# beecave-homelab/VibeVoice-ROCm

Measured on AMD Instinct MI355X. Metric: audio-sec/s, higher is better.
Workload: dtype bf16; 1 GPU; cfg2: VibeVoice-1.5B shapes, 1 speaker(s) x 203-frame voice prompt, 330-token prompt, 225 frames (30.0 s audio), CFG=2.0, 20 DPM-Solver++ steps, whole generate() incl. voice encode + prefill; global_batch=1, parallelism=replicas x1 (one dialogue per GPU), hipgraph=True

## Files before the change

vibevoice_rocm_amd/csrc/vv_fused.hip:

```cpp
#include <hip/hip_runtime.h>
#include <stdint.h>

#include "vv_hip.h"
#include "vv_common.h"
#include "vv_device.h"

namespace {

__device__ __forceinline__ float bf2f(bf16_t v) { return __uint_as_float((unsigned)v << 16); }
__device__ __forceinline__ float ldw(const float* p) { return *p; }
__device__ __forceinline__ float ldw(const bf16_t* p) { return bf2f(*p); }

template <typename WT>
__global__ __launch_bounds__(256) void head_init_kernel(const WT* P, const float* noise, int D, int latent, float* Xs, float* Ms, float* h0, int64_t ldh) {
  extern __shared__ float nz[];
  for (int i = threadIdx.x; i < latent; i += blockDim.x) nz[i] = noise[i];
  __syncthreads();
  const int n = blockIdx.x * blockDim.x + threadIdx.x;
  if (n >= D + latent) return;
  float s;
  if (n < D) {
    s = 0.f;
    const WT* pr = P + (int64_t)n * latent;
    for (int j = 0; j < latent; ++j) s = fmaf(ldw(pr + j), nz[j], s);
    h0[n] = s;
    h0[ldh + n] = s;
  } else {
    s = nz[n - D];
  }
  Xs[n] = s;
  Ms[n] = 0.f;
}

template <typename WT>
__global__ __launch_bounds__(256) void head_sde_proj_kernel(const WT* P, const float* noise, int64_t ld_noise, int n_steps, int D, int latent, float* NX) {
  extern __shared__ float nz[];
  const int u = blockIdx.y, N = D + latent;
  const float* nr = noise + (int64_t)(u / n_steps) * ld_noise + (int64_t)(u % n_steps) * latent;
  for (int i = threadIdx.x; i < latent; i += blockDim.x) nz[i] = nr[i];
  __syncthreads();
  const int n = blockIdx.x * blockDim.x + threadIdx.x;
  if (n >= N) return;
  float s;
  if (n < D) {
    s = 0.f;
    const WT* pr = P + (int64_t)n * latent;
    for (int j = 0; j < latent; ++j) s = fmaf(ldw(pr + j), nz[j], s);
  } else {
    s = nz[n - D];
  }
  NX[(int64_t)u * N + n] = s;
}

struct BoundaryArgs {
  const float* G;
  const float* h; int64_t ldh;
  const float* shift; const float* scale; int64_t ld_mod;
  float eps, cfg;
  vv_dpm_coef k;
  float* Xs; float* Ms;
  float* h_out; int64_t ldh_out;
  float* latent_out;
  int D, latent;
  int64_t state_stride, latent_stride;
  const float* nx; int64_t nx_stride;
};

template <int KU, bool SDE>
__global__ __launch_bounds__(256) void head_boundary_kernel(BoundaryArgs a) {
#include "vv_head_boundary.inc"
}

template <int KU, bool SDE>
__global__ __launch_bounds__(256) void head_boundary_cfg_kernel(BoundaryArgs a, const float* __restrict__ cfg_rows) {
  a.cfg = cfg_rows[blockIdx.y];
#include "vv_head_boundary.inc"
}

template <int KU> void launch_boundary(const BoundaryArgs& a, int B, hipStream_t s, const float* cfg_rows) {
  const int n = a.D + a.latent;
  int blocks = (n + 3) / 4;
  if (blocks > 512) blocks = 512;
  if (B > 1 && blocks > 256) blocks = 256;
  if (cfg_rows) {
    if (a.nx) hipLaunchKernelGGL((head_boundary_cfg_kernel<KU, true>), dim3(blocks, B), dim3(256), 0, s, a, cfg_rows);
    else hipLaunchKernelGGL((head_boundary_cfg_kernel<KU, false>), dim3(blocks, B), dim3(256), 0, s, a, cfg_rows);
    return;
  }
  if (a.nx) hipLaunchKernelGGL((head_boundary_kernel<KU, true>), dim3(blocks, B), dim3(256), 0, s, a);
  else hipLaunchKernelGGL((head_boundary_kernel<KU, false>), dim3(blocks, B), dim3(256), 0, s, a);
}

enum { TAIL_ARGMAX = 0, TAIL_SAMPLE = 1, TAIL_ROWS = 2 };

template <typename WT, bool SAMPLE>
__global__ __launch_bounds__(256) void llm_tail_kernel(const float* h, int64_t ldh, int R, int H, const float* norm_w, float eps, float* out, int64_t ldo,
                                                       const WT* w_valid, int nv, const int* ids, float* logits_out, int* token_out, const int* forced,
                                                       int* lens, int tok_start, int tok_diff, int* frame_ctr, const vv_sampler smp, const float* q) {
  constexpr int MODE = SAMPLE ? TAIL_SAMPLE : TAIL_ARGMAX;
  const vv_sampler* samplers = nullptr;
  const uint64_t* seeds = nullptr;
#include "vv_llm_tail.inc"
}

template <typename WT>
__global__ __launch_bounds__(256) void llm_tail_rows_kernel(const float* h, int64_t ldh, int R, int H, const float* norm_w, float eps, float* out, int64_t ldo,
                                                            const WT* w_valid, int nv, const int* ids, float* logits_out, int* token_out, const int* forced,
                                                            int* lens, int tok_start, int tok_diff, int* frame_ctr, const vv_sampler* __restrict__ samplers,
                                                            const uint64_t* __restrict__ seeds) {
  constexpr int MODE = TAIL_ROWS;
  const vv_sampler smp = {1.f, 0, 1.f};
  const float* q = nullptr;
#include "vv_llm_tail.inc"
}

template <typename WT, bool SAMPLE>
__global__ __launch_bounds__(256) void llm_tail_fast_kernel(const float* h, int64_t ldh, int R, int H, const float* norm_w, float eps, float* out, int64_t ldo,
                                                            const WT* w_valid, int nv, const int* ids, float* logits_out, int* token_out, const int* forced,
                                                            int* lens, int tok_start, int tok_diff, int* frame_ctr, const int* active,
                                                            const vv_sampler smp, const float* q) {
  constexpr int MODE = SAMPLE ? TAIL_SAMPLE : TAIL_ARGMAX;
  const vv_sampler* samplers = nullptr;
  const uint64_t* seeds = nullptr;
#include "vv_llm_tail_fast.inc"
}

template <typename WT>
__global__ __launch_bounds__(256) void llm_tail_fast_rows_kernel(const float* h, int64_t ldh, int R, int H, const float* norm_w, float eps, float* out,
                                                                 int64_t ldo, const WT* w_valid, int nv, const int* ids, float* logits_out, int* token_out,
                                                                 const int* forced, int* lens, int tok_start, int tok_diff, int* frame_ctr, const int* active,
                                                                 const vv_sampler* __restrict__ samplers, const uint64_t* __restrict__ seeds) {
  constexpr int MODE = TAIL_ROWS;
  const vv_sampler smp = {1.f, 0, 1.f};
  const float* q = nullptr;
#include "vv_llm_tail_fast.inc"
}

struct CtxItem { float* pad; float* state; int ctx, T, C; const float* dw_w; float* hs; int affine; float scale, bias; };
struct CtxArgs { CtxItem it[VV_MAX_STAGES + 1 + 16]; int n; };

__global__ __launch_bounds__(256) void conv_ctx_gather_kernel(const CtxArgs a) {
  const CtxItem it = a.it[blockIdx.y];
  const int n = it.ctx * it.C;
  if (it.affine) {
    for (int i = blockIdx.x * 256 + threadIdx.x; i < n; i += gridDim.x * 256) it.pad[i] = fmaf(it.state[i], it.scale, it.bias);
    return;
  }
  for (int i = (blockIdx.x * 256 + threadIdx.x) * 4; i < n; i += gridDim.x * 1024) {
    if (i + 3 < n && (n & 3) == 0) *reinterpret_cast<float4*>(it.pad + i) = *reinterpret_cast<const float4*>(it.state + i);
    else for (int j = i; j < n && j < i + 4; ++j) it.pad[j] = it.state[j];
  }
}
__global__ __launch_bounds__(256) void conv_ctx_scatter_kernel(const CtxArgs a) {
  const CtxItem it = a.it[blockIdx.y];
  const int n = it.ctx * it.C;
  const float* src = it.pad + (int64_t)it.T * it.C;
  for (int i = (blockIdx.x * 256 + threadIdx.x) * 4; i < n; i += gridDim.x * 1024) {
    if (i + 3 < n && (n & 3) == 0 && (((int64_t)it.T * it.C) & 3) == 0) *reinterpret_cast<float4*>(it.state + i) = *reinterpret_cast<const float4*>(src + i);
    else for (int j = i; j < n && j < i + 4; ++j) it.state[j] = src[j];
  }
  if (it.hs) {
    for (int c = blockIdx.x * 256 + threadIdx.x; c < it.C; c += gridDim.x * 256) {
      float s = 0.f;
#pragma unroll
      for (int k = 0; k < 6; ++k) s = fmaf(it.dw_w[(size_t)c * 7 + k], src[(size_t)k * it.C + c], s);
      it.hs[c] = s;
    }
  }
}


struct AdaTab { const bf16_t* w[17]; float* out[17]; int nblk[17]; int ldo[17]; int n; };

typedef __bf16 ad_bf16x8 __attribute__((ext_vector_type(8)));
typedef unsigned int ad_u32x4 __attribute__((ext_vector_type(4)));

template <int NST, int NM>
__global__ __launch_bounds__(256) void adaln_all_kernel(const bf16_t* __restrict__ c, int rows, int D, const AdaTab tab) {
  __shared__ float red[4 * NM * 4 * 64];
  const int tid = threadIdx.x, lane = tid & 63, wave = tid >> 6;
  int bx = blockIdx.x, l = 0;
  while (l + 1 < tab.n && bx >= tab.nblk[l]) { bx -= tab.nblk[l]; ++l; }
  const int n0 = bx * 16, m0 = blockIdx.y * (16 * NM);
  const int r16 = lane & 15, kq = lane >> 4;
  const int kb = wave * (32 * NST) + 8 * kq;
  const bf16_t* wr = tab.w[l] + (int64_t)(n0 + r16) * D + kb;
  ad_u32x4 wf[NST], xf[NM][NST];
#pragma unroll
  for (int s = 0; s < NST; ++s) wf[s] = *reinterpret_cast<const ad_u32x4*>(wr + 32 * s);
#pragma unroll
  for (int t = 0; t < NM; ++t) {
    const bf16_t* xr = c + (int64_t)min(m0 + 16 * t + r16, rows - 1) * D + kb;
#pragma unroll
    for (int s = 0; s < NST; ++s) xf[t][s] = *reinterpret_cast<const ad_u32x4*>(xr + 32 * s);
  }
  f32x4 acc[NM];
#pragma unroll
  for (int t = 0; t < NM; ++t) acc[t] = f32x4{0.f, 0.f, 0.f, 0.f};
#pragma unroll
  for (int s = 0; s < NST; ++s)
#pragma unroll
    for (int t = 0; t < NM; ++t)
      acc[t] = __builtin_amdgcn_mfma_f32_16x16x32_bf16(__builtin_bit_cast(ad_bf16x8, wf[s]), __builtin_bit_cast(ad_bf16x8, xf[t][s]), acc[t], 0, 0, 0);
#pragma unroll
  for (int t = 0; t < NM; ++t)
#pragma unroll
    for (int i = 0; i < 4; ++i) red[((wave * NM + t) * 4 + i) * 64 + lane] = acc[t][i];
  __syncthreads();
  const int ei = tid >> 6, el = tid & 63;
  float* out = tab.out[l];
  const int ldo = tab.ldo[l];
#pragma unroll
  for (int t = 0; t < NM; ++t) {
    const int m = m0 + 16 * t + (el & 15);
    if (m < rows) {
      float v = 0.f;
#pragma unroll
      for (int w4 = 0; w4 < 4; ++w4) v += red[((w4 * NM + t) * 4 + ei) * 64 + el];
      out[(int64_t)m * ldo + n0 + 4 * (el >> 4) + ei] = v;
    }
  }
}

template <int NST>
__global__ __launch_bounds__(256) void adaln_lds_kernel(const bf16_t* __restrict__ c, int rows, const AdaTab tab, int total) {
  constexpr int D = 4 * 32 * NST, P = D + 8, NM = 3, RG = 40;
  extern __shared__ __attribute__((aligned(16))) unsigned char ad_smem[];
  bf16_t* xs = reinterpret_cast<bf16_t*>(ad_smem);
  const int tid = threadIdx.x, lane = tid & 63, wave = tid >> 6;
  const int m0 = blockIdx.y * RG;
  const int nr = min(RG, rows - m0);
  float* red = reinterpret_cast<float*>(ad_smem + (size_t)RG * P * 2);
  const int r16 = lane & 15, kq = lane >> 4;
// ... 165 lines not shown
      if (ch < KU * 128) {
        const float4 v = tv[r][c], w = nv[r][c];
        *reinterpret_cast<float4*>(&ys[r][ch * 4]) = ch < nchunks ? make_float4(v.x * rs * w.x, v.y * rs * w.y, v.z * rs * w.z, v.w * rs * w.w) : make_float4(0.f, 0.f, 0.f, 0.f);
      }
    }
  }
  asm volatile("s_waitcnt lgkmcnt(0)\n\ts_barrier" ::: "memory");
  float ya[KU][8], yb[KU][8];
#pragma unroll
  for (int u = 0; u < KU; ++u) {
#pragma unroll
    for (int h2 = 0; h2 < 2; ++h2) {
      const float4 p = *reinterpret_cast<const float4*>(&ys[0][u * 512 + lane * 8 + 4 * h2]), q = *reinterpret_cast<const float4*>(&ys[1][u * 512 + lane * 8 + 4 * h2]);
      ya[u][4 * h2] = p.x; ya[u][4 * h2 + 1] = p.y; ya[u][4 * h2 + 2] = p.z; ya[u][4 * h2 + 3] = p.w;
      yb[u][4 * h2] = q.x; yb[u][4 * h2 + 1] = q.y; yb[u][4 * h2 + 2] = q.z; yb[u][4 * h2 + 3] = q.w;
    }
  }
  for (int i = 0; i < rows_per_wave; ++i) {
    const int row = gw + i * nwaves;
    float sa = 0.f, sb = 0.f;
#pragma unroll
    for (int u = 0; u < KU; ++u) {
      const unsigned ua[4] = {wa[u].x, wa[u].y, wa[u].z, wa[u].w}, ub[4] = {wsm[u].x, wsm[u].y, wsm[u].z, wsm[u].w};
#pragma unroll
      for (int j = 0; j < 4; ++j) {
        sa = fmaf(__uint_as_float(ua[j] << 16), ya[u][2 * j], sa); sa = fmaf(__uint_as_float(ua[j] & 0xffff0000u), ya[u][2 * j + 1], sa);
        sb = fmaf(__uint_as_float(ub[j] << 16), yb[u][2 * j], sb); sb = fmaf(__uint_as_float(ub[j] & 0xffff0000u), yb[u][2 * j + 1], sb);
      }
    }
    if (i + 1 < rows_per_wave) issue(row + nwaves);
    sa = vv_wave_sum(sa);
    sb = vv_wave_sum(sb);
    if (lane == 0 && row < H) {
      const float v = (sa + a.b2_a[row]) + (sb + a.b2_s[row]);
      for (int r = 0; r < a.rows_out; ++r) a.out[(int64_t)r * a.ldo + row] = v;
    }
  }
}


struct HeadPreArgs {
  const bf16_t* Wc; const float* cond; int64_t ld_cond; int K;
  const float* temb; int n_steps; bf16_t* c_out;
  const bf16_t* P; const float* noise; int D, latent; float* Xs; float* Ms; float* h0; int64_t ldh;
  int gemv_blocks;
};

template <int KU>
__global__ __launch_bounds__(256) void head_pre_kernel(const HeadPreArgs a) {
  const int tid = threadIdx.x, lane = tid & 63, wave = tid >> 6;
  if ((int)blockIdx.x >= a.gemv_blocks) {
    __shared__ float nz[256];
    for (int i = tid; i < a.latent; i += 256) nz[i] = a.noise[i];
    __syncthreads();
    const int n = ((int)blockIdx.x - a.gemv_blocks) * 256 + tid;
    if (n >= a.D + a.latent) return;
    float s;
    if (n < a.D) {
      s = 0.f;
      const bf16_t* pr = a.P + (int64_t)n * a.latent;
      for (int j = 0; j < a.latent; ++j) s = fmaf(bf2f(pr[j]), nz[j], s);
      a.h0[n] = s;
      a.h0[a.ldh + n] = s;
    } else {
      s = nz[n - a.D];
    }
    a.Xs[n] = s;
    a.Ms[n] = 0.f;
    return;
  }
  const int D = a.D, npairs = D >> 1;
  const int nwaves = a.gemv_blocks * 4;
  int g = blockIdx.x * 4 + wave;
  float x[2][KU][8];
#pragma unroll
  for (int r = 0; r < 2; ++r)
#pragma unroll
    for (int u = 0; u < KU; ++u) {
      const float4 p = *reinterpret_cast<const float4*>(a.cond + r * a.ld_cond + u * 512 + lane * 8), q = *reinterpret_cast<const float4*>(a.cond + r * a.ld_cond + u * 512 + lane * 8 + 4);
      x[r][u][0] = p.x; x[r][u][1] = p.y; x[r][u][2] = p.z; x[r][u][3] = p.w; x[r][u][4] = q.x; x[r][u][5] = q.y; x[r][u][6] = q.z; x[r][u][7] = q.w;
    }
  for (; g < npairs; g += nwaves) {
    const int n = 2 * g;
    uint4 w[2][KU];
#pragma unroll
    for (int o = 0; o < 2; ++o)
#pragma unroll
      for (int u = 0; u < KU; ++u) w[o][u] = *reinterpret_cast<const uint4*>(a.Wc + (int64_t)(n + o) * a.K + u * 512 + lane * 8);
    float te[2][2];
#pragma unroll
    for (int ps = 0; ps < 2; ++ps) {
      const int i = min(lane + 64 * ps, a.n_steps - 1);
      const float2 t2 = *reinterpret_cast<const float2*>(a.temb + (int64_t)i * D + n);
      te[ps][0] = t2.x; te[ps][1] = t2.y;
    }
    float acc[2][2];
#pragma unroll
    for (int o = 0; o < 2; ++o) {
      acc[o][0] = 0.f; acc[o][1] = 0.f;
#pragma unroll
      for (int u = 0; u < KU; ++u) {
        const unsigned uu[4] = {w[o][u].x, w[o][u].y, w[o][u].z, w[o][u].w};
#pragma unroll
        for (int j = 0; j < 4; ++j) {
          const float w0 = __uint_as_float(uu[j] << 16), w1 = __uint_as_float(uu[j] & 0xffff0000u);
          acc[o][0] = fmaf(w0, x[0][u][2 * j], acc[o][0]); acc[o][0] = fmaf(w1, x[0][u][2 * j + 1], acc[o][0]);
          acc[o][1] = fmaf(w0, x[1][u][2 * j], acc[o][1]); acc[o][1] = fmaf(w1, x[1][u][2 * j + 1], acc[o][1]);
        }
      }
    }
    float c0[2][2];
#pragma unroll
    for (int o = 0; o < 2; ++o)
#pragma unroll
      for (int r = 0; r < 2; ++r) c0[o][r] = vv_wave_sum(acc[o][r]);
#pragma unroll
    for (int ps = 0; ps < 2; ++ps) {
      const int i = lane + 64 * ps;
      if (i < a.n_steps) {
#pragma unroll
        for (int r = 0; r < 2; ++r) {
          const float v0 = c0[0][r] + te[ps][0], v1 = c0[1][r] + te[ps][1];
          *reinterpret_cast<unsigned*>(a.c_out + ((int64_t)(i * 2 + r)) * D + n) = bf16_bits2(vv_silu(v0), vv_silu(v1));
        }
      }
    }
  }
}

}

int vv_head_init_fused(const vv_head* h, const float* noise, float* Xs, float* Ms, float* h0, int64_t ldh, hipStream_t s) {
  const int n = h->D + h->latent;
  const int blocks = (n + 255) / 256;
  const size_t lds = (size_t)h->latent * sizeof(float);
  if (h->wdt == VV_F32) hipLaunchKernelGGL((head_init_kernel<float>), dim3(blocks), dim3(256), lds, s, (const float*)h->noisy_proj, noise, h->D, h->latent, Xs, Ms, h0, ldh);
  else hipLaunchKernelGGL((head_init_kernel<bf16_t>), dim3(blocks), dim3(256), lds, s, (const bf16_t*)h->noisy_proj, noise, h->D, h->latent, Xs, Ms, h0, ldh);
  VV_CHECK_LAUNCH("vv_head_init_fused");
  return 0;
}

int vv_head_sde_proj_fused(const vv_head* h, const float* sde_noise, int64_t ld_sde, int n_steps, int B, float* NX, hipStream_t s) {
  const int n = h->D + h->latent;
  const dim3 grid((n + 255) / 256, B * n_steps);
  const size_t lds = (size_t)h->latent * sizeof(float);
  if (h->wdt == VV_F32)
    hipLaunchKernelGGL((head_sde_proj_kernel<float>), grid, dim3(256), lds, s, (const float*)h->noisy_proj, sde_noise, ld_sde, n_steps, h->D, h->latent, NX);
  else
    hipLaunchKernelGGL((head_sde_proj_kernel<bf16_t>), grid, dim3(256), lds, s, (const bf16_t*)h->noisy_proj, sde_noise, ld_sde, n_steps, h->D, h->latent, NX);
  VV_CHECK_LAUNCH("vv_head_sde_proj_fused");
  return 0;
}

bool vv_head_boundary_supported(const vv_head* h) {
  return h->fused_g != nullptr && h->D % 8 == 0 && h->D <= 4096 && ((uintptr_t)h->fused_g % 16 == 0);
}

int vv_head_boundary_decide(const vv_head* h) {
  const int ku = (h->D + 511) / 512;
  return (h->D > 0 && ku <= 8) ? ku : 0;
}

int vv_head_boundary_fused(const vv_head* h, const float* hrows, int64_t ldh, const float* shift, const float* scale, int64_t ld_mod, float cfg,
                           const vv_dpm_coef* k, float* Xs, float* Ms, float* h_out, int64_t ldh_out, float* latent_out, hipStream_t s) {
  return vv_head_boundary_batch(h, hrows, ldh, shift, scale, ld_mod, cfg, k, Xs, Ms, 0, h_out, ldh_out, latent_out, 0, 1, s);
}

int vv_head_boundary_batch(const vv_head* h, const float* hrows, int64_t ldh, const float* shift, const float* scale, int64_t ld_mod, float cfg,
                           const vv_dpm_coef* k, float* Xs, float* Ms, int64_t state_stride, float* h_out, int64_t ldh_out, float* latent_out,
                           int64_t latent_stride, int B, hipStream_t s, const float* nx, int64_t nx_stride, const float* cfg_rows) {
  BoundaryArgs a;
  a.state_stride = state_stride; a.latent_stride = latent_stride;
  a.nx = k->cn != 0.f ? nx : nullptr; a.nx_stride = nx_stride;
  a.G = h->fused_g; a.h = hrows; a.ldh = ldh; a.shift = shift; a.scale = scale; a.ld_mod = ld_mod; a.eps = h->eps; a.cfg = cfg; a.k = *k;
  a.Xs = Xs; a.Ms = Ms; a.h_out = h_out; a.ldh_out = ldh_out; a.latent_out = latent_out; a.D = h->D; a.latent = h->latent;
  switch (vv_head_boundary_decide(h)) {
    case 1: launch_boundary<1>(a, B, s, cfg_rows); break;
    case 2: launch_boundary<2>(a, B, s, cfg_rows); break;
    case 3: launch_boundary<3>(a, B, s, cfg_rows); break;
    case 4: launch_boundary<4>(a, B, s, cfg_rows); break;
    case 5: launch_boundary<5>(a, B, s, cfg_rows); break;
    case 6: launch_boundary<6>(a, B, s, cfg_rows); break;
    case 7: launch_boundary<7>(a, B, s, cfg_rows); break;
    case 8: launch_boundary<8>(a, B, s, cfg_rows); break;
    default: return vv_set_error(VV_E_UNSUPPORTED, "vv_head_boundary_fused: D=%d", h->D);
  }
  VV_CHECK_LAUNCH("vv_head_boundary_fused");
  return 0;
}

static int check_sampler(const char* name, const vv_sampler* smp, const float* q, int nv) {
  if (!smp || !q) return vv_set_error(VV_E_ARG, "%s: null sampler / q", name);
  if (!(smp->temperature > 0.f) || !(smp->top_p > 0.f && smp->top_p <= 1.f)) return vv_set_error(VV_E_ARG, "%s: temperature=%g (> 0) top_p=%g (0 < top_p <= 1)", name, (double)smp->temperature, (double)smp->top_p);
  if (nv > 8) return vv_set_error(VV_E_ARG, "%s: nv=%d (<= 8)", name, nv);
  return 0;
}

#define VV_TAIL_FAST(WT, SAMPLE, grid, R_, act)                                                                                                          \
  hipLaunchKernelGGL((llm_tail_fast_kernel<WT, SAMPLE>), dim3(grid), dim3(256), 0, s, h, ldh, R_, m->hidden, m->final_norm, m->rms_eps, out, ldo, (const WT*)w_valid, nv, \
                     ids, logits_out, token_out, forced_token, lens, tok_start, tok_diffusion, frame_counter, act, sv, q)
#define VV_TAIL_GEN(WT, SAMPLE)                                                                                                                         \
  hipLaunchKernelGGL((llm_tail_kernel<WT, SAMPLE>), dim3(1), dim3(256), lds, s, h, ldh, R, m->hidden, m->final_norm, m->rms_eps, out, ldo, (const WT*)w_valid, nv, ids, \
                     logits_out, token_out, forced_token, lens, tok_start, tok_diffusion, frame_counter, sv, q)
#define VV_TAIL_FAST_ROWS(WT, grid, R_, act)                                                                                                             \
  hipLaunchKernelGGL((llm_tail_fast_rows_kernel<WT>), dim3(grid), dim3(256), 0, s, h, ldh, R_, m->hidden, m->final_norm, m->rms_eps, out, ldo, (const WT*)w_valid, nv, \
                     ids, logits_out, token_out, forced_token, lens, tok_start, tok_diffusion, frame_counter, act, rows, seeds)
#define VV_TAIL_GEN_ROWS(WT)                                                                                                                            \
  hipLaunchKernelGGL((llm_tail_rows_kernel<WT>), dim3(1), dim3(256), lds, s, h, ldh, R, m->hidden, m->final_norm, m->rms_eps, out, ldo, (const WT*)w_valid, nv, ids, \
                     logits_out, token_out, forced_token, lens, tok_start, tok_diffusion, frame_counter, rows, seeds)

static int llm_tail_launch(const char* name, const vv_llm* m, const float* h, int64_t ldh, int R, float* out, int64_t ldo, const void* w_valid, int nv, const int* ids,
                           float* logits_out, int* token_out, const int* forced_token, int* lens, int tok_start, int tok_diffusion, int* frame_counter,
                           const vv_sampler* smp, const float* q, hipStream_t s, const vv_sampler* rows = nullptr, const uint64_t* seeds = nullptr) {
  const vv_sampler sv = smp ? *smp : vv_sampler{1.f, 0, 1.f};
  const size_t lds = (size_t)m->hidden * sizeof(float);
  auto a16 = [](const void* p) { return ((uintptr_t)p % 16) == 0; };
  if (R <= 2 && nv <= 8 && m->hidden % 4 == 0 && m->hidden <= 4096 && a16(h) && ldh % 4 == 0 && a16(out) && ldo % 4 == 0 && a16(m->final_norm) &&
      ((uintptr_t)w_valid % (m->wdt == VV_F32 ? 16 : 8)) == 0 && (m->wdt == VV_F32 || m->hidden % 4 == 0)) {
    if (rows) { if (m->wdt == VV_F32) VV_TAIL_FAST_ROWS(float, 1, R, (const int*)nullptr); else VV_TAIL_FAST_ROWS(bf16_t, 1, R, (const int*)nullptr); }
    else if (m->wdt == VV_F32) { if (smp) VV_TAIL_FAST(float, true, 1, R, (const int*)nullptr); else VV_TAIL_FAST(float, false, 1, R, (const int*)nullptr); }
    else { if (smp) VV_TAIL_FAST(bf16_t, true, 1, R, (const int*)nullptr); else VV_TAIL_FAST(bf16_t, false, 1, R, (const int*)nullptr); }
    VV_CHECK_LAUNCH(name);
    return 0;
  }
  if (rows) { if (m->wdt == VV_F32) VV_TAIL_GEN_ROWS(float); else VV_TAIL_GEN_ROWS(bf16_t); }
  else if (m->wdt == VV_F32) { if (smp) VV_TAIL_GEN(float, true); else VV_TAIL_GEN(float, false); }
  else { if (smp) VV_TAIL_GEN(bf16_t, true); else VV_TAIL_GEN(bf16_t, false); }
  VV_CHECK_LAUNCH(name);
  return 0;
}

static int llm_tail_batch_launch(const char* name, const vv_llm* m, const float* h, int64_t ldh, int B, float* out, int64_t ldo, const void* w_valid, int nv,
                                 const int* ids, float* logits_out, int* token_out, const int* forced_token, int* lens, int tok_start, int tok_diffusion,
                                 int* frame_counter, const int* active, const vv_sampler* smp, const float* q, hipStream_t s,
                                 const vv_sampler* rows = nullptr, const uint64_t* seeds = nullptr) {
  const vv_sampler sv = smp ? *smp : vv_sampler{1.f, 0, 1.f};
  auto a16 = [](const void* p) { return ((uintptr_t)p % 16) == 0; };
  if (!(m->hidden % 4 == 0 && m->hidden <= 4096 && a16(h) && ldh % 4 == 0 && a16(out) && ldo % 4 == 0 && a16(m->final_norm) &&
        ((uintptr_t)w_valid % (m->wdt == VV_F32 ? 16 : 8)) == 0))
    return vv_set_error(VV_E_UNSUPPORTED, "%s: hidden=%d / alignment not covered", name, m->hidden);
  if (rows) { if (m->wdt == VV_F32) VV_TAIL_FAST_ROWS(float, B, 2, active); else VV_TAIL_FAST_ROWS(bf16_t, B, 2, active); }
  else if (m->wdt == VV_F32) { if (smp) VV_TAIL_FAST(float, true, B, 2, active); else VV_TAIL_FAST(float, false, B, 2, active); }
  else { if (smp) VV_TAIL_FAST(bf16_t, true, B, 2, active); else VV_TAIL_FAST(bf16_t, false, B, 2, active); }
  VV_CHECK_LAUNCH(name);
  return 0;
}
#undef VV_TAIL_FAST
#undef VV_TAIL_GEN
#undef VV_TAIL_FAST_ROWS
#undef VV_TAIL_GEN_ROWS

extern "C" int vv_llm_tail(const vv_llm* m, const float* h, int64_t ldh, int R, float* out, int64_t ldo, const void* w_valid, int nv, const int* ids,
                           float* logits_out, int* token_out, const int* forced_token, int* lens, int tok_start, int tok_diffusion,
                           int* frame_counter, vv_stream_t stream) {
  if (!m || !h || !out || !w_valid || !ids || !logits_out || !token_out) return vv_set_error(VV_E_ARG, "vv_llm_tail: null pointer");
  if (R <= 0 || nv <= 0 || nv > 16) return vv_set_error(VV_E_ARG, "vv_llm_tail: R=%d nv=%d (nv <= 16)", R, nv);
  return llm_tail_launch("vv_llm_tail", m, h, ldh, R, out, ldo, w_valid, nv, ids, logits_out, token_out, forced_token, lens, tok_start, tok_diffusion, frame_counter,
                         nullptr, nullptr, (hipStream_t)stream);
}

extern "C" int vv_llm_tail_sample(const vv_llm* m, const float* h, int64_t ldh, int R, float* out, int64_t ldo, const void* w_valid, int nv, const int* ids,
                                  float* logits_out, int* token_out, const int* forced_token, int* lens, int tok_start, int tok_diffusion,
                                  int* frame_counter, const vv_sampler* sampler, const float* q, vv_stream_t stream) {
  if (!m || !h || !out || !w_valid || !ids || !logits_out || !token_out) return vv_set_error(VV_E_ARG, "vv_llm_tail_sample: null pointer");
  if (R <= 0 || nv <= 0) return vv_set_error(VV_E_ARG, "vv_llm_tail_sample: R=%d nv=%d", R, nv);
  VV_TRY(check_sampler("vv_llm_tail_sample", sampler, q, nv));
  return llm_tail_launch("vv_llm_tail_sample", m, h, ldh, R, out, ldo, w_valid, nv, ids, logits_out, token_out, forced_token, lens, tok_start, tok_diffusion,
                         frame_counter, sampler, q, (hipStream_t)stream);
}

extern "C" int vv_llm_tail_batch(const vv_llm* m, const float* h, int64_t ldh, int B, float* out, int64_t ldo, const void* w_valid, int nv, const int* ids,
                                 float* logits_out, int* token_out, const int* forced_token, int* lens, int tok_start, int tok_diffusion,
                                 int* frame_counter, const int* active, vv_stream_t stream) {
  if (!m || !h || !out || !w_valid || !ids || !logits_out || !token_out) return vv_set_error(VV_E_ARG, "vv_llm_tail_batch: null pointer");
  if (B <= 0 || B > 8 || nv <= 0 || nv > 8) return vv_set_error(VV_E_ARG, "vv_llm_tail_batch: B=%d (1..8) nv=%d (<= 8)", B, nv);
  return llm_tail_batch_launch("vv_llm_tail_batch", m, h, ldh, B, out, ldo, w_valid, nv, ids, logits_out, token_out, forced_token, lens, tok_start, tok_diffusion,
                               frame_counter, active, nullptr, nullptr, (hipStream_t)stream);
}

extern "C" int vv_llm_tail_batch_sample(const vv_llm* m, const float* h, int64_t ldh, int B, float* out, int64_t ldo, const void* w_valid, int nv, const int* ids,
                                        float* logits_out, int* token_out, const int* forced_token, int* lens, int tok_start, int tok_diffusion,
                                        int* frame_counter, const int* active, const vv_sampler* sampler, const float* q, vv_stream_t stream) {
  if (!m || !h || !out || !w_valid || !ids || !logits_out || !token_out) return vv_set_error(VV_E_ARG, "vv_llm_tail_batch_sample: null pointer");
  if (B <= 0 || B > 8 || nv <= 0) return vv_set_error(VV_E_ARG, "vv_llm_tail_batch_sample: B=%d (1..8) nv=%d", B, nv);
  VV_TRY(check_sampler("vv_llm_tail_batch_sample", sampler, q, nv));
  return llm_tail_batch_launch("vv_llm_tail_batch_sample", m, h, ldh, B, out, ldo, w_valid, nv, ids, logits_out, token_out, forced_token, lens, tok_start,
                               tok_diffusion, frame_counter, active, sampler, q, (hipStream_t)stream);
}

extern "C" int vv_llm_tail_sample_rows(const vv_llm* m, const float* h, int64_t ldh, int R, float* out, int64_t ldo, const void* w_valid, int nv, const int* ids,
                                       float* logits_out, int* token_out, const int* forced_token, int* lens, int tok_start, int tok_diffusion,
                                       int* frame_counter, const vv_sampler* samplers, const uint64_t* seeds, vv_stream_t stream) {
  if (!m || !h || !out || !w_valid || !ids || !logits_out || !token_out) return vv_set_error(VV_E_ARG, "vv_llm_tail_sample_rows: null pointer");
  if (R <= 0 || nv <= 0 || nv > 8) return vv_set_error(VV_E_ARG, "vv_llm_tail_sample_rows: R=%d nv=%d (<= 8)", R, nv);
  if (!lens || !samplers || !seeds) return vv_set_error(VV_E_ARG, "vv_llm_tail_sample_rows: null lens / samplers / seeds");
  return llm_tail_launch("vv_llm_tail_sample_rows", m, h, ldh, R, out, ldo, w_valid, nv, ids, logits_out, token_out, forced_token, lens, tok_start, tok_diffusion,
                         frame_counter, nullptr, nullptr, (hipStream_t)stream, samplers, seeds);
}

extern "C" int vv_llm_tail_batch_sample_rows(const vv_llm* m, const float* h, int64_t ldh, int B, float* out, int64_t ldo, const void* w_valid, int nv,
                                             const int* ids, float* logits_out, int* token_out, const int* forced_token, int* lens, int tok_start,
                                             int tok_diffusion, int* frame_counter, const int* active, const vv_sampler* samplers, const uint64_t* seeds,
                                             vv_stream_t stream) {
  if (!m || !h || !out || !w_valid || !ids || !logits_out || !token_out) return vv_set_error(VV_E_ARG, "vv_llm_tail_batch_sample_rows: null pointer");
  if (B <= 0 || B > 8 || nv <= 0 || nv > 8) return vv_set_error(VV_E_ARG, "vv_llm_tail_batch_sample_rows: B=%d (1..8) nv=%d (<= 8)", B, nv);
  if (!lens || !samplers || !seeds) return vv_set_error(VV_E_ARG, "vv_llm_tail_batch_sample_rows: null lens / samplers / seeds");
// ... 115 lines not shown
```

vibevoice_rocm_amd/csrc/vv_kernels.hip:

```cpp
#include <hip/hip_runtime.h>
#include <hip/hip_bf16.h>
#include <stdint.h>
#include <stdio.h>
#include <string.h>
#include <math.h>

#include "vv_hip.h"
#include "vv_common.h"
#include "vv_device.h"

static thread_local char g_err[512] = "";

int vv_set_error(int code, const char* fmt, ...) {
  va_list ap;
  va_start(ap, fmt);
  vsnprintf(g_err, sizeof(g_err), fmt, ap);
  va_end(ap);
  return code;
}

extern "C" const char* vv_last_error(void) { return g_err; }
extern "C" int vv_abi_version(void) { return 6; }
int vv_mixer_init();
extern "C" int vv_init(void) {
  VV_TRY(vv_mixer_init());
  VV_TRY(vv_mfma_gemm_init());
  VV_TRY(vv_gemm_packed_init());
  VV_TRY(vv_block1d_init());
  VV_TRY(vv_convffn_init());
  VV_TRY(vv_gemv_rows_init());
  return vv_fused_init();
}
static float* g_rows_part = nullptr;
static int* g_rows_tk = nullptr;
static const size_t G_ROWS_PART_FLOATS = (size_t)4 << 20, G_ROWS_TICKETS = 4096;
static int rows_scratch(int on) {
  if (on && !g_rows_part) {
    if (hipMalloc(&g_rows_part, G_ROWS_PART_FLOATS * sizeof(float)) != hipSuccess || hipMalloc(&g_rows_tk, G_ROWS_TICKETS * sizeof(int)) != hipSuccess ||
        hipMemset(g_rows_tk, 0, G_ROWS_TICKETS * sizeof(int)) != hipSuccess)
      return vv_set_error(VV_E_HIP, "vv_tune: gemv_rows_scratch allocation failed");
  }
  if (!on && g_rows_part) { (void)hipFree(g_rows_part); (void)hipFree(g_rows_tk); g_rows_part = nullptr; g_rows_tk = nullptr; }
  return 0;
}
void vv_gemv_rows_set_dbg(int d);
void vv_gemv_rows_set_atomic(int on);
void vv_gemv_stream_set_blocks(int b);
void vv_gemv_stream_set_waves(int w);
void vv_gemv_stream_set_opt(int o);
void vv_gemv_stream_set_long(int cap, int ku);
void vv_gemv_stream_set_dual_rw(int r);
void vv_gemv_stream_set_small_rw(int r);
void vv_mfma_set_mt(int mt);
void vv_mfma_set_tiled_rows(int r);
void vv_mfma_set_tiled_bk128(int on);
void vv_mfma_set_tiled_small(int t);
void vv_mfma_set_tiled_dual_bk64(int on);
void vv_mfma_set_tiled_small_dual(int t);
void vv_mfma_set_tiled_small_k(int k);
void vv_mixer_set_rows(int on);
void vv_mfma_set_mt_prefill(int mt);
extern int g_attn_group;
void vv_attn_decode_set_gqa(int on);
void vv_attn_decode_set_gqa_keys(int k);
extern "C" int vv_tune(const char* key, int value) {
  if (key && !strcmp(key, "gemv_long_cap")) { vv_gemv_stream_set_long(value, 0); return 0; }
  if (key && !strcmp(key, "gemv_long_ku")) { vv_gemv_stream_set_long(0, value); return 0; }
  if (key && !strcmp(key, "gemv_blocks")) { vv_gemv_stream_set_blocks(value); vv_gemv_mx6_set_blocks(value); return 0; }
  if (key && !strcmp(key, "gemv_waves")) { vv_gemv_stream_set_waves(value); return 0; }
  if (key && !strcmp(key, "gemv_rows")) { vv_gemv_rows_set(value, 0, -1); return 0; }
  if (key && !strcmp(key, "gemv_rows_blocks")) { vv_gemv_rows_set(-1, value, -1); return 0; }
  if (key && !strcmp(key, "gemv_rows_pers")) { vv_gemv_rows_set(-1, 0, value); return 0; }
  if (key && !strcmp(key, "gemv_rows_scratch")) return rows_scratch(value);
  if (key && !strcmp(key, "gemv_rows_dbg")) { vv_gemv_rows_set_dbg(value); return 0; }
  if (key && !strcmp(key, "gemv_rows_atomic")) { vv_gemv_rows_set_atomic(value); return 0; }
  if (key && !strcmp(key, "gemv_opt")) { vv_gemv_stream_set_opt(value); return 0; }
  if (key && !strcmp(key, "gemv_dual_rw")) { vv_gemv_stream_set_dual_rw(value); return 0; }
  if (key && !strcmp(key, "gemv_small_rw")) { vv_gemv_stream_set_small_rw(value); return 0; }
  if (key && !strcmp(key, "gemv_hot")) { vv_gemv_hot_set(value); return 0; }
  if (key && !strcmp(key, "conv_hot")) { vv_conv_hot_set(value); return 0; }
  if (key && !strcmp(key, "mixer_rows")) { vv_mixer_set_rows(value); return 0; }
  if (key && !strcmp(key, "block1d_fused")) { vv_block1d_set_fused(value); return 0; }
  if (key && !strcmp(key, "block1d_blocks")) { vv_block1d_set_blocks(value); return 0; }
  if (key && !strcmp(key, "convffn")) { vv_convffn_set(value); return 0; }
  if (key && !strcmp(key, "convffn_t1")) { vv_convffn_set_t1(value); return 0; }
  if (key && !strcmp(key, "convffn_t1hs")) { vv_convffn_set_t1hs(value); return 0; }
  if (key && !strcmp(key, "convffn_rows512")) { vv_convffn_set_rows(512, value); return 0; }
  if (key && !strcmp(key, "convffn_rows256")) { vv_convffn_set_rows(256, value); return 0; }
  if (key && !strcmp(key, "convffn_rows128")) { vv_convffn_set_rows(128, value); return 0; }
  if (key && !strcmp(key, "convffn_c128")) { vv_convffn_set_c128(value); return 0; }
  if (key && !strcmp(key, "skinny")) { vv_skinny_set(value, 0, 0); return 0; }
  if (key && !strcmp(key, "skinny_min_m")) { vv_skinny_set(1, value, 0); return 0; }
  if (key && !strcmp(key, "skinny_max_m")) { vv_skinny_set(1, 0, value); return 0; }
  if (key && !strcmp(key, "mfma_tiled_bk128")) { vv_mfma_set_tiled_bk128(value); return 0; }
  if (key && !strcmp(key, "attn_group")) { g_attn_group = value; return 0; }
  if (key && !strcmp(key, "attn_gqa")) { vv_attn_decode_set_gqa(value); return 0; }
  if (key && !strcmp(key, "attn_gqa_keys")) { vv_attn_decode_set_gqa_keys(value); return 0; }
  if (key && !strcmp(key, "mfma_tiled_small_k")) { vv_mfma_set_tiled_small_k(value); return 0; }
  if (key && !strcmp(key, "mfma_tiled_dual_bk64")) { vv_mfma_set_tiled_dual_bk64(value); return 0; }
  if (key && !strcmp(key, "mfma_tiled_small_dual")) { vv_mfma_set_tiled_small_dual(value); return 0; }
  if (key && !strcmp(key, "mfma_tiled_small")) { vv_mfma_set_tiled_small(value); return 0; }
  if (key && !strcmp(key, "mfma_tiled_rows")) { vv_mfma_set_tiled_rows(value); return 0; }
  if (key && !strcmp(key, "gemm_packed_rows")) { vv_gemm_packed_set_rows(value); return 0; }
  if (key && !strcmp(key, "mfma_mt")) { vv_mfma_set_mt(value); return 0; }
  if (key && !strcmp(key, "mfma_mt_prefill")) { vv_mfma_set_mt_prefill(value); return 0; }
  return vv_set_error(VV_E_ARG, "vv_tune: unknown key");
}

__device__ __forceinline__ float bf2f(unsigned int u16) { return __uint_as_float(u16 << 16); }
__device__ __forceinline__ float wave_sum(float v) {
#pragma unroll
  for (int o = 32; o > 0; o >>= 1) v += __shfl_xor(v, o);
  return v;
}

template <typename WT> struct WL;
template <> struct WL<float> {
  static __device__ __forceinline__ void load8(const float* p, float (&o)[8]) {
    const float4 a = *reinterpret_cast<const float4*>(p);
    const float4 b = *reinterpret_cast<const float4*>(p + 4);
    o[0] = a.x; o[1] = a.y; o[2] = a.z; o[3] = a.w; o[4] = b.x; o[5] = b.y; o[6] = b.z; o[7] = b.w;
  }
  static __device__ __forceinline__ void load4(const float* p, float (&o)[4]) {
    const float4 a = *reinterpret_cast<const float4*>(p);
    o[0] = a.x; o[1] = a.y; o[2] = a.z; o[3] = a.w;
  }
  static __device__ __forceinline__ float load1(const float* p) { return *p; }
};
template <> struct WL<bf16_t> {
  static __device__ __forceinline__ void load8(const bf16_t* p, float (&o)[8]) {
    const uint4 v = *reinterpret_cast<const uint4*>(p);
    unpack8(u32x4{v.x, v.y, v.z, v.w}, o);
  }
  static __device__ __forceinline__ void load4(const bf16_t* p, float (&o)[4]) {
    const uint2 v = *reinterpret_cast<const uint2*>(p);
    o[0] = __uint_as_float(v.x << 16); o[1] = __uint_as_float(v.x & 0xffff0000u);
    o[2] = __uint_as_float(v.y << 16); o[3] = __uint_as_float(v.y & 0xffff0000u);
  }
  static __device__ __forceinline__ float load1(const bf16_t* p) { return bf2f(*p); }
};

__device__ __forceinline__ void lin_epilogue(const vv_lin_args& a, int m, int n, float v, float v2) {
  a.out[(int64_t)m * a.ldo + n] = vv_epi_value(a, v, v2, EpiAtUse{a, m, n});
}

#define GEMV_THREADS 256

template <int M>
__device__ __forceinline__ void row_stats(const vv_lin_args& a, float* red, float (&rstd)[M]) {
  const int tid = threadIdx.x, lane = tid & 63, wave = tid >> 6;
  float ss[M];
#pragma unroll
  for (int m = 0; m < M; ++m) {
    const float* xr = a.x + (int64_t)m * a.ldx;
    float s = 0.f;
    for (int k = tid; k < a.k; k += GEMV_THREADS) { const float v = xr[k]; s += v * v; }
    ss[m] = wave_sum(s);
  }
  if (lane == 0) {
#pragma unroll
    for (int m = 0; m < M; ++m) red[wave * M + m] = ss[m];
  }
  __syncthreads();
#pragma unroll
  for (int m = 0; m < M; ++m) {
    const float t = red[m] + red[M + m] + red[2 * M + m] + red[3 * M + m];
    rstd[m] = rsqrtf(t / (float)a.k + a.eps);
  }
  __syncthreads();
}

template <int M>
__device__ __forceinline__ void stage_chunk(const vv_lin_args& a, float* xs, int kc0, int kc, int kcp, const float (&rstd)[M]) {
  for (int idx = threadIdx.x; idx < M * kcp; idx += GEMV_THREADS) {
    const int m = idx / kcp, kk = idx - m * kcp;
    float v = 0.f;
    if (kk < kc) {
      const int k = kc0 + kk;
      v = a.x[(int64_t)m * a.ldx + k];
      if (a.pro == VV_PRO_RMSNORM) {
        v *= rstd[m];
        if (a.norm_w) v *= a.norm_w[k];
        if (a.mod_scale) v = v * (1.0f + a.mod_scale[(int64_t)m * a.ld_mod + k]) + a.mod_shift[(int64_t)m * a.ld_mod + k];
      } else if (a.pro == VV_PRO_SILU) {
        v = vv_silu(v);
      }
    }
    xs[idx] = v;
  }
}

template <typename WT, int M, bool DUAL, int KSPLIT, int RW>
__global__ __launch_bounds__(GEMV_THREADS) void gemv_kernel(const vv_lin_args a, const int KC) {
  extern __shared__ __attribute__((aligned(16))) float smem[];
  float* red = smem;
  float* xs = smem + 64 * 4;
  const int tid = threadIdx.x, lane = tid & 63, wave = tid >> 6;
  const int K = a.k, N = a.n;
  const WT* __restrict__ W = reinterpret_cast<const WT*>(a.w);
  const WT* __restrict__ W2 = reinterpret_cast<const WT*>(a.w2);

  float rstd[M];
#pragma unroll
  for (int m = 0; m < M; ++m) rstd[m] = 1.f;
  if (a.pro == VV_PRO_RMSNORM) row_stats<M>(a, red, rstd);

  const int row0 = (KSPLIT == 1 ? (blockIdx.x * 4 + wave) : blockIdx.x) * RW;
  float acc[RW][M], acc2[DUAL ? RW : 1][M];
#pragma unroll
  for (int r = 0; r < RW; ++r)
#pragma unroll
    for (int m = 0; m < M; ++m) { acc[r][m] = 0.f; if (DUAL) acc2[r][m] = 0.f; }

  for (int kc0 = 0; kc0 < K; kc0 += KC) {
    const int kc = min(KC, K - kc0);
    const int kcp = (kc + 7) & ~7;
    if (kc0 > 0) __syncthreads();
    stage_chunk<M>(a, xs, kc0, kc, kcp, rstd);
    __syncthreads();
    const int kstart = (KSPLIT == 1 ? lane : (wave * 64 + lane)) * 8;
    const int kstep = (KSPLIT == 1 ? 64 : 256) * 8;
#pragma unroll 2
    for (int k = kstart; k < kc; k += kstep) {
      float w[RW][8], w2[DUAL ? RW : 1][8];
#pragma unroll
      for (int r = 0; r < RW; ++r) {
        const int n = min(row0 + r, N - 1);
        WL<WT>::load8(W + (int64_t)n * K + kc0 + k, w[r]);
        if (DUAL) WL<WT>::load8(W2 + (int64_t)n * K + kc0 + k, w2[r]);
      }
#pragma unroll
      for (int m = 0; m < M; ++m) {
        const float4 x0 = *reinterpret_cast<const float4*>(xs + m * kcp + k);
        const float4 x1 = *reinterpret_cast<const float4*>(xs + m * kcp + k + 4);
        const float xv[8] = {x0.x, x0.y, x0.z, x0.w, x1.x, x1.y, x1.z, x1.w};
#pragma unroll
        for (int r = 0; r < RW; ++r) {
#pragma unroll
          for (int j = 0; j < 8; ++j) {
            acc[r][m] = fmaf(w[r][j], xv[j], acc[r][m]);
            if (DUAL) acc2[r][m] = fmaf(w2[r][j], xv[j], acc2[r][m]);
          }
        }
      }
    }
  }
#pragma unroll
  for (int r = 0; r < RW; ++r)
#pragma unroll
    for (int m = 0; m < M; ++m) { acc[r][m] = wave_sum(acc[r][m]); if (DUAL) acc2[r][m] = wave_sum(acc2[r][m]); }
// ... 1776 lines not shown
```

Measured before the change: 44.07 audio-sec/s.

## Add multi-row specialized head boundary kernel for D=1536 single-batch CFG

Adds a specialized diffusion-head boundary kernel for D=1536, latent=64, B=1 with shared CFG and no SDE noise. Each wave computes two output rows and issues all of its weight loads before the RMSNorm/CFG stage. The grid is sized to exactly (D+latent)/8 blocks. The intent is to cut per-block fixed work and hide weight-load latency behind the normalization. In exchange it adds a shape-specific code path with more register pressure, and relies on the row count dividing evenly (1600/8=200).

```diff
diff --git a/vibevoice_rocm_amd/csrc/vv_fused.hip b/vibevoice_rocm_amd/csrc/vv_fused.hip
--- a/vibevoice_rocm_amd/csrc/vv_fused.hip
+++ b/vibevoice_rocm_amd/csrc/vv_fused.hip
@@ -77,8 +77,124 @@
 #include "vv_head_boundary.inc"
 }
 
+template <int R>
+__global__ __launch_bounds__(256) void head_boundary_rows_kernel(BoundaryArgs a) {
+  constexpr int KU = 3, NCH = (KU * 128 + 255) / 256;
+  __shared__ __attribute__((aligned(16))) float ys[KU * 512];
+  __shared__ float red[4][2];
+  const int tid = threadIdx.x, lane = tid & 63, wave = tid >> 6;
+  const int D = a.D;
+  const int nchunks = D >> 2;
+  float4 hv[2][NCH], sv[2][NCH], cv[2][NCH];
+#pragma unroll
+  for (int c = 0; c < NCH; ++c) {
+    const int ch = tid + c * 256;
+    const int kk = ch < nchunks ? ch * 4 : 0;
+#pragma unroll
+    for (int r = 0; r < 2; ++r) {
+      hv[r][c] = *reinterpret_cast<const float4*>(a.h + r * a.ldh + kk);
+      sv[r][c] = *reinterpret_cast<const float4*>(a.shift + r * a.ld_mod + kk);
+      cv[r][c] = *reinterpret_cast<const float4*>(a.scale + r * a.ld_mod + kk);
+    }
+  }
+  const int gstride = gridDim.x * 4;
+  const int g = blockIdx.x * 4 + wave;
+  float4 w[R][KU][2];
+  float xs[R], ms[R];
+#pragma unroll
+  for (int i = 0; i < R; ++i) {
+    const float* gr = a.G + (int64_t)(g + i * gstride) * D + lane * 8;
+#pragma unroll
+    for (int u = 0; u < KU; ++u) {
+      w[i][u][0] = *reinterpret_cast<const float4*>(gr + u * 512);
+      w[i][u][1] = *reinterpret_cast<const float4*>(gr + u * 512 + 4);
+    }
+  }
+#pragma unroll
+  for (int i = 0; i < R; ++i) { xs[i] = a.Xs[g + i * gstride]; ms[i] = a.Ms[g + i * gstride]; }
+  __builtin_amdgcn_sched_barrier(0);
+#pragma unroll
+  for (int c = 0; c < NCH; ++c)
+#pragma unroll
+    for (int r = 0; r < 2; ++r) { VV_FENCE4(hv[r][c]); VV_FENCE4(sv[r][c]); VV_FENCE4(cv[r][c]); }
+  float ss[2];
+#pragma unroll
+  for (int r = 0; r < 2; ++r) {
+    float s1 = 0.f;
+#pragma unroll
+    for (int c = 0; c < NCH; ++c) {
+      const float4 v = hv[r][c];
+      s1 += (tid + c * 256 < nchunks) ? (v.x * v.x + v.y * v.y) + (v.z * v.z + v.w * v.w) : 0.f;
+    }
+    ss[r] = vv_wave_sum(s1);
+  }
+  if (lane == 0) { red[wave][0] = ss[0]; red[wave][1] = ss[1]; }
+  __syncthreads();
+  {
+    const float rs0 = rsqrtf(((red[0][0] + red[1][0]) + (red[2][0] + red[3][0])) / (float)D + a.eps);
+    const float rs1 = rsqrtf(((red[0][1] + red[1][1]) + (red[2][1] + red[3][1])) / (float)D + a.eps);
+#pragma unroll
+    for (int c = 0; c < NCH; ++c) {
+      const int ch = tid + c * 256;
+      if (ch < KU * 128) {
+        float4 y = make_float4(0.f, 0.f, 0.f, 0.f);
+        if (ch < nchunks) {
+          const float4 h0 = hv[0][c], h1 = hv[1][c];
+          const float yc0 = h0.x * rs0 * (1.0f + cv[0][c].x) + sv[0][c].x, yu0 = h1.x * rs1 * (1.0f + cv[1][c].x) + sv[1][c].x;
+          const float yc1 = h0.y * rs0 * (1.0f + cv[0][c].y) + sv[0][c].y, yu1 = h1.y * rs1 * (1.0f + cv[1][c].y) + sv[1][c].y;
+          const float yc2 = h0.z * rs0 * (1.0f + cv[0][c].z) + sv[0][c].z, yu2 = h1.z * rs1 * (1.0f + cv[1][c].z) + sv[1][c].z;
+          const float yc3 = h0.w * rs0 * (1.0f + cv[0][c].w) + sv[0][c].w, yu3 = h1.w * rs1 * (1.0f + cv[1][c].w) + sv[1][c].w;
+          y = make_float4(yu0 + a.cfg * (yc0 - yu0), yu1 + a.cfg * (yc1 - yu1), yu2 + a.cfg * (yc2 - yu2), yu3 + a.cfg * (yc3 - yu3));
+        }
+        *reinterpret_cast<float4*>(&ys[ch * 4]) = y;
+      }
+    }
+  }
+  __syncthreads();
+  float yr[KU][8];
+#pragma unroll
+  for (int u = 0; u < KU; ++u) {
+    const float4 p = *reinterpret_cast<const float4*>(&ys[u * 512 + lane * 8]);
+    const float4 q = *reinterpret_cast<const float4*>(&ys[u * 512 + lane * 8 + 4]);
+    yr[u][0] = p.x; yr[u][1] = p.y; yr[u][2] = p.z; yr[u][3] = p.w; yr[u][4] = q.x; yr[u][5] = q.y; yr[u][6] = q.z; yr[u][7] = q.w;
+  }
+#pragma unroll
+  for (int i = 0; i < R; ++i) {
+    const int gi = g + i * gstride;
+    float acc = 0.f;
+#pragma unroll
+    for (int u = 0; u < KU; ++u) {
+      const float wr[8] = {w[i][u][0].x, w[i][u][0].y, w[i][u][0].z, w[i][u][0].w, w[i][u][1].x, w[i][u][1].y, w[i][u][1].z, w[i][u][1].w};
+#pragma unroll
+      for (int j = 0; j < 8; ++j) acc = fmaf(wr[j], yr[u][j], acc);
+    }
+    const float z = vv_wave_sum(acc);
+    if (lane == 0) {
+      const float x0 = a.k.alpha_s * xs[i] - a.k.sigma_s * z;
+      float xt = a.k.cx * xs[i] - a.k.cd * x0;
+      if (a.k.order == 2) xt -= 0.5f * a.k.cd * (a.k.rinv * (x0 - ms[i]));
+      a.Xs[gi] = xt;
+      a.Ms[gi] = x0;
+      if (gi < D) { a.h_out[gi] = xt; a.h_out[a.ldh_out + gi] = xt; }
+      else a.latent_out[gi - D] = xt;
+    }
+  }
+}
+
+constexpr int BOUNDARY_ROWS_DEFAULT = 2;
+int g_boundary_rows = BOUNDARY_ROWS_DEFAULT;
+
+int boundary_rows_decide(int D, int latent, int B, bool per_utterance_cfg, bool sde) {
+  const int r = g_boundary_rows;
+  return (D == 1536 && latent == 64 && B == 1 && !per_utterance_cfg && !sde && r == BOUNDARY_ROWS_DEFAULT) ? r : 0;
+}
+
 template <int KU> void launch_boundary(const BoundaryArgs& a, int B, hipStream_t s, const float* cfg_rows) {
   const int n = a.D + a.latent;
+  if (const int rows = boundary_rows_decide(a.D, a.latent, B, cfg_rows != nullptr, a.nx != nullptr)) {
+    hipLaunchKernelGGL((head_boundary_rows_kernel<BOUNDARY_ROWS_DEFAULT>), dim3(n / (4 * rows)), dim3(256), 0, s, a);
+    return;
+  }
   int blocks = (n + 3) / 4;
   if (blocks > 512) blocks = 512;
   if (B > 1 && blocks > 256) blocks = 256;
@@ -550,6 +666,9 @@
   return 0;
 }
 
+void vv_head_boundary_set_rows(int r) { g_boundary_rows = r < 0 ? BOUNDARY_ROWS_DEFAULT : r; }
+extern "C" int vv_head_boundary_rows(int D, int latent, int B, int per_utterance_cfg, int sde) { return boundary_rows_decide(D, latent, B, per_utterance_cfg != 0, sde != 0); }
+
 bool vv_head_boundary_supported(const vv_head* h) {
   return h->fused_g != nullptr && h->D % 8 == 0 && h->D <= 4096 && ((uintptr_t)h->fused_g % 16 == 0);
 }
diff --git a/vibevoice_rocm_amd/csrc/vv_kernels.hip b/vibevoice_rocm_amd/csrc/vv_kernels.hip
--- a/vibevoice_rocm_amd/csrc/vv_kernels.hip
+++ b/vibevoice_rocm_amd/csrc/vv_kernels.hip
@@ -63,6 +63,7 @@
 extern int g_attn_group;
 void vv_attn_decode_set_gqa(int on);
 void vv_attn_decode_set_gqa_keys(int k);
+void vv_head_boundary_set_rows(int r);
 extern "C" int vv_tune(const char* key, int value) {
   if (key && !strcmp(key, "gemv_long_cap")) { vv_gemv_stream_set_long(value, 0); return 0; }
   if (key && !strcmp(key, "gemv_long_ku")) { vv_gemv_stream_set_long(0, value); return 0; }
@@ -96,6 +97,7 @@
   if (key && !strcmp(key, "attn_group")) { g_attn_group = value; return 0; }
   if (key && !strcmp(key, "attn_gqa")) { vv_attn_decode_set_gqa(value); return 0; }
   if (key && !strcmp(key, "attn_gqa_keys")) { vv_attn_decode_set_gqa_keys(value); return 0; }
+  if (key && !strcmp(key, "head_boundary_rows")) { vv_head_boundary_set_rows(value); return 0; }
   if (key && !strcmp(key, "mfma_tiled_small_k")) { vv_mfma_set_tiled_small_k(value); return 0; }
   if (key && !strcmp(key, "mfma_tiled_dual_bk64")) { vv_mfma_set_tiled_dual_bk64(value); return 0; }
   if (key && !strcmp(key, "mfma_tiled_small_dual")) { vv_mfma_set_tiled_small_dual(value); return 0; }
```

Result: no change. 44.29 audio-sec/s, median of 6 (+0.5%).
